# openai/gym

Measured on AMD Instinct MI355X. Metric: env-steps/sec at num_envs=2^20, CartPole-v1, higher is better.
Workload: dtype f64

## Files before the change

### gym_amd/_native.py

```python
from __future__ import annotations

import ctypes as C
import os
import sys
import weakref

import numpy as np

_HERE = os.path.dirname(os.path.abspath(__file__))
LIB_PATH = os.environ.get("MXV_LIB_PATH") or os.path.join(_HERE, "_lib", "libmxv.so")

CARTPOLE, PENDULUM, ACROBOT, MOUNTAINCAR, MOUNTAINCAR_CONT = range(5)
FLAG_ACTION_I32 = 1
FLAG_REWARD_F32 = 2
FLAG_NO_AUTORESET = 4
OK = 0
ERR_INVALID_ARG = -1
ERR_HIP = -2
ERR_INVALID_ACTION = -3
ERR_RESET_NEEDED = -4
ERR_UNSUPPORTED = -5
MAX_PARAMS = 12
ENV_ALIGN = 4
ROLLOUT_EAGER, ROLLOUT_GRAPH, ROLLOUT_FUSED = 0, 1, 2
TAB_FLAG_COMPACT = 1
TAB_FLAG_GENERAL_KERNEL = 2
TAB_KERNEL_NONE, TAB_KERNEL_GENERAL, TAB_KERNEL_TRAJECTORY = 0, 1, 2
COMM_ID_BYTES = 128

EXPORTS = (
    "mxv_env_dims", "mxv_default_params", "mxv_default_reset_bounds", "mxv_version", "mxv_create", "mxv_destroy",
    "mxv_last_error", "mxv_seed", "mxv_seed_actions", "mxv_reset", "mxv_step", "mxv_step_sampled", "mxv_rollout",
    "mxv_rollout_tape", "mxv_sample_actions", "mxv_last_launch", "mxv_last_launch_snapshot", "mxv_reset_host", "mxv_step_host", "mxv_get_state", "mxv_set_state", "mxv_get_counters",
    "mxv_set_counters", "mxv_set_device_clock", "mxv_set_obs_partials", "mxv_set_return_partials", "mxv_obs_partials_layout", "mxv_get_episodes", "mxv_set_episodes", "mxv_get_params", "mxv_set_params", "mxv_set_params_per_env", "mxv_get_params_per_env", "mxv_episode_stats", "mxv_set_episode_outputs", "mxv_episode_stats_host", "mxv_set_running_returns", "mxv_sync", "mxv_get_stream", "mxv_set_stream",
    "mxv_rollout_mixed", "mxv_set_final_snapshot", "mxv_comm_unique_id", "mxv_comm_init", "mxv_comm_destroy", "mxv_allgather_outputs", "mxv_allgather_wait", "mxv_comm_stream",
    "mxv_host_io", "mxv_step_mapped", "mxv_reset_mapped", "mxv_final_packed", "mxv_final_packed_view", "mxv_final_packed_stats_view", "mxv_write_probe", "mxv_write_probe_env", "mxv_host_alloc", "mxv_host_free",
                "mxv_host_block_layout", "mxv_step_host_block", "mxv_wait_stream", "mxv_staging_view", "mxv_adopt_obs",
    "mxv_norm_create", "mxv_norm_destroy", "mxv_norm_last_error", "mxv_norm_set_stream", "mxv_norm_get_state",
    "mxv_norm_set_state", "mxv_norm_observations", "mxv_norm_rewards", "mxv_norm_obs_sums", "mxv_norm_obs_sums_partials", "mxv_norm_reward_sums_partials", "mxv_norm_returns_ptr", "mxv_norm_obs_apply",
    "mxv_norm_reward_sums", "mxv_norm_reward_apply",
    "mxv_subnorm_create", "mxv_subnorm_destroy", "mxv_subnorm_last_error", "mxv_subnorm_set_stream", "mxv_subnorm_get_state",
    "mxv_subnorm_set_state", "mxv_subnorm_observations", "mxv_subnorm_rewards",
    "mxv_tab_create", "mxv_tab_destroy", "mxv_tab_last_error", "mxv_tab_seed", "mxv_tab_seed_actions", "mxv_tab_reset",
    "mxv_tab_step", "mxv_tab_rollout", "mxv_tab_rollout_tape", "mxv_tab_reset_host", "mxv_tab_step_host", "mxv_tab_get_state",
    "mxv_tab_set_state", "mxv_tab_episode_stats", "mxv_tab_set_episode_outputs", "mxv_tab_episode_stats_host",
    "mxv_bj_episode_stats", "mxv_bj_set_episode_outputs", "mxv_bj_episode_stats_host", "mxv_tab_set_running_returns", "mxv_bj_set_running_returns", "mxv_tab_get_counters", "mxv_tab_set_counters", "mxv_tab_sync", "mxv_tab_last_kernel", "mxv_tab_word_threshold", "mxv_tab_set_device_clock", "mxv_bj_set_device_clock", "mxv_tab_set_stream",
    "mxv_get_beyond", "mxv_set_beyond",
    "mxv_bj_create", "mxv_bj_destroy", "mxv_bj_last_error", "mxv_bj_seed", "mxv_bj_reset", "mxv_bj_step", "mxv_bj_rollout", "mxv_bj_rollout_compact",
    "mxv_bj_reset_host", "mxv_bj_step_host", "mxv_bj_get_state", "mxv_bj_set_state", "mxv_bj_get_counters", "mxv_bj_sync", "mxv_bj_set_stream",
    "mxv_placed_alloc", "mxv_placed_free", "mxv_placed_info_get", "mxv_placed_last_error", "mxv_hbm_pair_probe",
)


class MxvLaunchInfo(C.Structure):
    _fields_ = [(k, C.c_int32) for k in ("kernel", "env_id", "param_mode", "envs_per_lane", "safe", "out_mode", "tape", "steps")] + \
               [("grid", C.c_uint32), ("block", C.c_uint32)]
# ... 100 lines not shown
        raise ImportError(
            f"{LIB_PATH} is missing: build the HIP extension first (python -c 'import __graft_entry__ as g; g.build()' "
            "or gym_amd/csrc/build.sh). gym_amd has no CPU fallback."
        )
    _share_torch_hip_runtime()
    lib = C.CDLL(LIB_PATH)
    vp, i32, i64, u64, u32 = C.c_void_p, C.c_int32, C.c_int64, C.c_uint64, C.c_uint32
    sig = {
        "mxv_env_dims": ([i32, C.POINTER(i32), C.POINTER(i32), C.POINTER(i32)], C.c_int),
        "mxv_default_params": ([i32, vp], C.c_int),
        "mxv_default_reset_bounds": ([i32, vp], C.c_int),
        "mxv_version": ([], C.c_char_p),
        "mxv_create": ([C.POINTER(MxvConfig), C.POINTER(vp)], C.c_int),
        "mxv_seed": ([vp, u64, vp], C.c_int),
        "mxv_seed_actions": ([vp, u64], C.c_int),
        "mxv_reset": ([vp, vp, vp, vp], C.c_int),
        "mxv_step": ([vp, vp, vp, vp, vp, vp, vp], C.c_int),
        "mxv_step_sampled": ([vp, vp, vp, vp, vp, vp, vp], C.c_int),
        "mxv_rollout": ([vp, i32, i32, i32, vp, vp, vp, vp, vp, vp], C.c_int),
        "mxv_rollout_tape": ([vp, i32, i32, vp, vp, vp, vp, vp, vp], C.c_int),
        "mxv_sample_actions": ([vp, vp], C.c_int),
        "mxv_last_launch": ([vp, C.POINTER(MxvLaunchInfo)], C.c_int),
        "mxv_last_launch_snapshot": ([vp, C.POINTER(i32), C.POINTER(i32)], C.c_int),
        "mxv_reset_host": ([vp, vp, vp, vp], C.c_int),
        "mxv_step_host": ([vp, vp, vp, vp, vp, vp, vp], C.c_int),
        "mxv_get_state": ([vp, vp, vp], C.c_int),
        "mxv_adopt_obs": ([vp, vp], C.c_int),
        "mxv_set_state": ([vp, vp, vp], C.c_int),
        "mxv_set_counters": ([vp, u64, u32], C.c_int),
        "mxv_set_obs_partials": ([vp, vp], C.c_int),
        "mxv_set_return_partials": ([vp, vp, C.c_double, vp], C.c_int),
        "mxv_obs_partials_layout": ([vp, C.POINTER(i64), C.POINTER(i64), C.POINTER(i32)], C.c_int),
        "mxv_rollout_mixed": ([vp, C.c_int32, C.c_int32, C.c_int32, vp], C.c_int),
        "mxv_set_final_snapshot": ([vp, vp, vp, vp, vp], C.c_int),
        "mxv_write_probe": ([C.c_int32, i64, C.c_int32, C.c_int32, vp, vp, vp, vp, vp, C.POINTER(C.c_double)], C.c_int),
        "mxv_write_probe_env": ([C.c_int32, C.c_int32, C.c_int32, i64, C.c_int32, C.c_int32, vp, vp, vp, vp, vp, C.POINTER(C.c_double)], C.c_int),
        "mxv_wait_stream": ([vp, vp], C.c_int),
        "mxv_staging_view": ([vp] + [C.POINTER(vp)] * 4, C.c_int),
        "mxv_host_alloc": ([C.c_size_t, C.POINTER(vp)], C.c_int),
        "mxv_host_free": ([vp], C.c_int),
        "mxv_host_block_layout": ([vp] + [C.POINTER(C.c_size_t)] * 6, C.c_int),
        "mxv_step_host_block": ([vp, vp, vp, C.c_int32], C.c_int),
        "mxv_final_packed": ([vp, C.c_int32, C.POINTER(C.c_int32)], C.c_int),
        "mxv_final_packed_stats_view": ([vp, C.POINTER(vp), C.POINTER(vp)], C.c_int),
        "mxv_final_packed_view": ([vp, C.POINTER(vp), C.POINTER(vp), C.POINTER(vp)], C.c_int),
        "mxv_comm_unique_id": ([vp], C.c_int),
# ... 485 lines not shown

    def get_state(self):
        st = np.empty((self.S, self.num_envs), dtype=np.float64)
        el = np.empty(self.num_envs, dtype=np.int32)
        self._check(lib.mxv_get_state(self._h, st.ctypes.data, el.ctypes.data))
        return st, el

    def set_state(self, state=None, elapsed=None):
        st = None if state is None else np.ascontiguousarray(state, dtype=np.float64)
        el = None if elapsed is None else np.ascontiguousarray(elapsed, dtype=np.int32)
        if st is not None:
            assert st.shape == (self.S, self.num_envs), st.shape
        if el is not None:
            assert el.shape == (self.num_envs,)
        self._check(lib.mxv_set_state(self._h, _ptr(st), _ptr(el)))

    def last_launch(self) -> dict:
        info = MxvLaunchInfo()
        self._check(lib.mxv_last_launch(self._h, C.byref(info)))
        out = {k: int(getattr(info, k)) for k, _ in MxvLaunchInfo._fields_}
        out["snapshot"] = int(self._final_snapshot()[1])
        return out

    def _final_snapshot(self):
        attached, deposited = C.c_int32(), C.c_int32()
        self._check(lib.mxv_last_launch_snapshot(self._h, C.byref(attached), C.byref(deposited)))
        return bool(attached.value), bool(deposited.value)

    @property
    def final_snapshot_attached(self) -> bool:
        return self._final_snapshot()[0]

    def set_counters(self, t: int, r: int):
        self._check(lib.mxv_set_counters(self._h, int(t), int(r)))

    def set_obs_partials(self, partials_dev=None):
        self._check(lib.mxv_set_obs_partials(self._h, _ptr(partials_dev)))

    def set_return_partials(self, returns_state_ptr=None, gamma: float = 0.99, partials_dev=None):
        self._check(lib.mxv_set_return_partials(self._h, _ptr(returns_state_ptr), float(gamma), _ptr(partials_dev)))

    def obs_partials_layout(self):
        lv, per, vals = C.c_int64(), C.c_int64(), C.c_int32()
        self._check(lib.mxv_obs_partials_layout(self._h, C.byref(lv), C.byref(per), C.byref(vals)))
        return lv.value, per.value, vals.value

# ... 527 lines not shown
```

### gym_amd/csrc/mxv_api.cpp

```cpp
#include <hip/hip_runtime.h>
#include <dlfcn.h>
#include <rccl/rccl.h>

#include <algorithm>
#include <cmath>
#include <cstdlib>
#include <cstring>
#include <map>
#include <new>
#include <string>
#include <tuple>
#include <vector>

#include "mxv_host.hpp"
#include "mxv_kernels.hpp"
#include "mxv_render.hpp"
#include "../../include/mxv_render.h"

using namespace mxv;

namespace {

constexpr int kStateDim[MXV_NUM_ENV_KINDS] = {4, 2, 4, 2, 2};
constexpr int kObsDim[MXV_NUM_ENV_KINDS] = {4, 3, 6, 2, 2};
// ... 34 lines not shown

}

struct mxv_handle : mxv::HostCore {
    static constexpr const char *kNullMessage = "NULL handle";
    mxv_handle() : HostCore("mxv") {}
    mxv_config cfg{};
    int S = 0, O = 0, NA = 0;
    double *state = nullptr;
    float *adopted_obs = nullptr;
    int32_t *lo = nullptr;
    bool hilo = false;
    void *elapsed = nullptr;
    bool elapsed16 = false;
    uint32_t *episodes = nullptr;
    double *ret_state = nullptr, *ret_part = nullptr;
    double ret_gamma = 0.0;
    double *obs_part = nullptr;
    uint32_t *clock_ticket = nullptr;
    bool state_injected = false;
    bool state_out_of_range = false;
    LaunchInfo last_launch{-1, 0, 0, 0, 0, 0, 0, 0, 0, 0};
    bool last_launch_snapshot = false;
    bool step_noise = false;
    EnvParams P{};
    bool default_params = true;
    uint8_t *beyond = nullptr;
    double *params_pe = nullptr;
    int param_mode() const { return params_pe ? PM_PER_ENV : (default_params ? PM_DEFAULT : PM_BROADCAST); }
    double bounds[2] = {0, 0};
    void *st_actions = nullptr;
    float *st_obs = nullptr, *st_final = nullptr;
    void *st_reward = nullptr;
    uint8_t *st_term = nullptr, *st_trunc = nullptr, *st_mask = nullptr;
    void *hm_block = nullptr;
    void *dv_block = nullptr;
    size_t io_total = 0, io_out_off = 0, io_out_bytes = 0, io_act_bytes = 0;
    int32_t *hm_err = nullptr;
    bool hostmap = false;
    char *fin_dev = nullptr;
    char *fin_host = nullptr;
    bool err_in_block = false;
    size_t fin_last = 0;
    bool fin_packed = false;
    using GraphKey = std::tuple<int, int, void *, void *, void *, void *, void *, void *>;
    std::map<GraphKey, hipGraphExec_t> graphs;
// ... 54 lines not shown
    a.state = h->state;
    a.elapsed = h->elapsed;
    a.elapsed16 = h->elapsed16 ? 1 : 0;
    a.episodes = h->episodes;
    a.seeds = h->seeds;
    a.t_dev = nullptr;
    a.err = h->err_in_block ? h->hm_err : h->err;
    a.n = h->cfg.num_envs;
    a.env0 = (uint64_t)h->cfg.env_offset;
    a.base_seed = h->base_seed;
    a.action_seed = h->action_seed;
    a.t = h->t;
    if (h->dev_clock) {
        a.t_dev = h->t_dev;
        a.t = 0;
    }
    a.b0 = h->bounds[0];
    a.b1 = h->bounds[1];
    a.max_steps = h->cfg.max_episode_steps;
    a.flags = h->cfg.flags;
    a.K = 1;
    a.state_injected = (h->state_injected || h->state_out_of_range) ? 1 : 0;
    a.step_noise = h->step_noise ? 1 : 0;
    a.slice = 0;
    a.act_slice = 0;
    a.params_pe = h->params_pe;
    a.beyond = h->beyond;
    a.ep_acc = h->ep_acc;
    a.ep_return_out = h->ep_acc ? h->ep_return_out : nullptr;
    a.ep_length_out = h->ep_acc ? h->ep_length_out : nullptr;
    a.snap_obs = nullptr;
    a.snap_reward = nullptr;
    a.snap_terminated = a.snap_truncated = nullptr;
    a.P = h->P;
}

int track_source(mxv_handle *h, const void *actions, int64_t row, int32_t K, const float **src) {
    *src = nullptr;
    if (!h->last_u) return MXV_OK;
    if (actions) {
        *src = (const float *)actions + row * h->cfg.num_envs;
        return MXV_OK;
    }
    SampleArgs a{};
    a.actions_out = h->blit_actions;
    a.t_dev = h->dev_clock ? h->t_dev : nullptr;
// ... 83 lines not shown
    fill_step_args(h, a);
    a.actions = actions;
    a.actions_out = actions_out;
    a.obs = obs;
    a.reward = reward;
    a.terminated = term;
    a.truncated = trunc;
    a.final_obs = final_obs;
    const bool self_clock = h->dev_clock && h->cfg.num_envs <= kClockInKernelEnvs && h->param_mode() == PM_DEFAULT && !hilo_step;
    if (self_clock) {
        a.clock_out = h->t_dev;
        a.clock_ticket = h->clock_ticket;
    }
    if (int rc = check_step_buffers(h, a)) return rc;
    const float *track = nullptr;
    if (int rc = track_source(h, actions, 0, 1, &track)) return rc;
    if (hilo_step) {
        a.hi_in = h->adopted_obs;
        a.lo = h->lo;
        MXV_HIP(h, launch_hilo_step(h->cfg.env_id, a, h->stream, &h->last_launch));
    } else {
        MXV_HIP(h, launch_step(h->cfg.env_id, h->param_mode(), a, h->stream, &h->last_launch));
    }
    h->last_launch_snapshot = false;
    h->state_injected = false;
    if (int rc = track_step(h, track)) return rc;
    if (self_clock) {
        h->t += 1;
        return MXV_OK;
    }
    return clock_add(h, 1);
}

int parse_bounds(mxv_handle *h, const double *b, double *out) {
    if (!b) {
        default_bounds(h->cfg.env_id, out);
        return MXV_OK;
    }
    if (std::isnan(b[0]) || std::isnan(b[1])) return fail(h, MXV_ERR_INVALID_ARG, "reset bounds are NaN");
    if (h->cfg.env_id != MXV_PENDULUM && b[0] > b[1])
        return fail(h, MXV_ERR_INVALID_ARG, "Lower bound (%g) must be lower than higher bound (%g).", b[0], b[1]);
    out[0] = b[0];
    out[1] = b[1];
    return MXV_OK;
}

// ... 338 lines not shown
    if (h->obs_part || h->ret_part) {
        a.obs_part = h->obs_part;
        if (h->ret_part) {
            a.ret_part = h->ret_part;
            a.ret_state = h->ret_state;
            a.ret_gamma = h->ret_gamma;
        }
        if (!launch_step_supports_stats(h->cfg.env_id, h->param_mode(), a))
            return fail(h, MXV_ERR_UNSUPPORTED, "partial sums are attached (mxv_set_obs_partials / mxv_set_return_partials), but this launch cannot produce them: they "
                                                "exist for sampled [K][N] trajectory launches (K >= 2) with every per-step output, default physics "
                                                "parameters, autoreset and a state the engine produced itself; detach (NULL) and use mxv_norm_obs_sums / mxv_norm_reward_sums");
    }
    const bool in_kernel = h->snap_obs && launch_step_is_rollout(h->param_mode(), a);
    if (in_kernel) {
        a.snap_obs = h->snap_obs;
        a.snap_reward = h->snap_reward;
        a.snap_terminated = h->snap_term;
        a.snap_truncated = h->snap_trunc;
    }
    if (int rc = check_step_buffers(h, a)) return rc;
    const float *track = nullptr;
    if (int rc = track_source(h, actions_tape, K - 1, K, &track)) return rc;
    MXV_HIP(h, launch_step(h->cfg.env_id, h->param_mode(), a, h->stream, &h->last_launch));
    h->last_launch_snapshot = a.snap_obs != nullptr;
    h->state_injected = false;
    if (int rc = track_step(h, track)) return rc;
    if (int rc = clock_add(h, K)) return rc;
    if (h->snap_obs && !in_kernel) return copy_final_snapshot(h, K, per_step, obs, reward, term, trunc);
    return MXV_OK;
}

}

extern "C" {

int mxv_rollout(mxv_handle *h, int32_t K, int32_t per_step, int32_t mode, void *actions_out_dev, float *obs_dev,
                void *reward_dev, uint8_t *terminated_dev, uint8_t *truncated_dev, float *final_obs_dev) {
    MXV_CHECK(h);
    if (int rc = rollout_checks(h, K, obs_dev)) return rc;
    if (mode == MXV_ROLLOUT_FUSED)
        return fused_launch(h, K, per_step, nullptr, actions_out_dev, obs_dev, reward_dev, terminated_dev,
                            truncated_dev, final_obs_dev);
    if (mode != MXV_ROLLOUT_EAGER && mode != MXV_ROLLOUT_GRAPH) return fail(h, MXV_ERR_INVALID_ARG, "unknown rollout mode %d", mode);
    if (int rc = no_partials_here(h, "a rollout of single-step launches (MXV_ROLLOUT_EAGER / _GRAPH)")) return rc;
    const size_t n = (size_t)h->cfg.num_envs;
    auto slice = [&](void *p, size_t elem_bytes, int k) -> void * {
        if (!p) return nullptr;
        return per_step ? (void *)((char *)p + (size_t)k * n * elem_bytes) : p;
    };
    {
        StepArgs a0{};
        fill_step_args(h, a0);
        a0.actions_out = actions_out_dev; a0.obs = obs_dev; a0.reward = reward_dev; a0.final_obs = final_obs_dev;
        if (int rc = check_step_buffers(h, a0)) return rc;
    }
    auto launch_k = [&](int k, const uint64_t *t_dev, uint64_t t) -> hipError_t {
        StepArgs a{};
        fill_step_args(h, a);
        a.t_dev = t_dev;
        a.t = t;
        a.actions = nullptr;
        a.actions_out = slice(actions_out_dev, h->action_bytes(), k);
        a.obs = (float *)slice(obs_dev, h->O * sizeof(float), k);
        a.reward = slice(reward_dev, h->reward_bytes(), k);
        a.terminated = (uint8_t *)slice(terminated_dev, 1, k);
        a.truncated = (uint8_t *)slice(truncated_dev, 1, k);
        a.final_obs = (float *)slice(final_obs_dev, h->O * sizeof(float), k);
        a.ep_return_out = (float *)slice(a.ep_return_out, sizeof(float), k);
        a.ep_length_out = (int32_t *)slice(a.ep_length_out, sizeof(int32_t), k);
        return launch_step(h->cfg.env_id, h->param_mode(), a, h->stream, &h->last_launch);
    };
    const float *track = nullptr;
    if (int rc = track_source(h, nullptr, 0, K, &track)) return rc;
    hipStreamCaptureStatus capturing = hipStreamCaptureStatusNone;
    (void)hipStreamIsCapturing(h->stream, &capturing);
    if (mode == MXV_ROLLOUT_EAGER || capturing != hipStreamCaptureStatusNone) {
        for (int k = 0; k < K; ++k)
            MXV_HIP(h, launch_k(k, h->dev_clock ? h->t_dev : nullptr, h->dev_clock ? (uint64_t)k : h->t + (uint64_t)k));
    } else {
        mxv_handle::GraphKey key{K, per_step, actions_out_dev, obs_dev, reward_dev, terminated_dev, truncated_dev,
                                 final_obs_dev};
        auto it = h->graphs.find(key);
        if (it == h->graphs.end()) {
            hipGraph_t graph = nullptr;
            MXV_HIP(h, hipStreamBeginCapture(h->stream, hipStreamCaptureModeThreadLocal));
            hipError_t le = hipSuccess;
            for (int k = 0; k < K && le == hipSuccess; ++k) le = launch_k(k, h->t_dev, (uint64_t)k);
            hipError_t ce = hipStreamEndCapture(h->stream, &graph);
            if (le != hipSuccess || ce != hipSuccess) {
                if (graph) (void)hipGraphDestroy(graph);
                return fail(h, MXV_ERR_HIP, "graph capture: %s", hipGetErrorString(le != hipSuccess ? le : ce));
            }
// ... 354 lines not shown
                    in_range = false;
                    break;
                }
        }
        h->state_injected = !in_range;
        h->state_out_of_range = !in_range && h->cfg.env_id == MXV_PENDULUM;
    }
    return MXV_OK;
}

int mxv_last_launch(mxv_handle *h, mxv_launch_info *out) {
    MXV_CHECK(h);
    if (!out) return fail(h, MXV_ERR_INVALID_ARG, "mxv_last_launch: out is NULL");
    static_assert(sizeof(mxv_launch_info) == sizeof(LaunchInfo), "mxv_launch_info mirrors LaunchInfo member for member");
    std::memcpy(out, &h->last_launch, sizeof(*out));
    return MXV_OK;
}

int mxv_last_launch_snapshot(mxv_handle *h, int32_t *attached, int32_t *deposited) {
    MXV_CHECK(h);
    if (!attached && !deposited) return fail(h, MXV_ERR_INVALID_ARG, "mxv_last_launch_snapshot: both outputs are NULL");
    if (attached) *attached = h->snap_obs != nullptr ? 1 : 0;
    if (deposited) *deposited = h->last_launch_snapshot ? 1 : 0;
    return MXV_OK;
}

int mxv_get_counters(mxv_handle *h, uint64_t *t, uint32_t *r) {
    MXV_CHECK(h);
    return get_counters(h, t, r);
}

int mxv_set_counters(mxv_handle *h, uint64_t t, uint32_t r) {
    MXV_CHECK(h);
    return set_counters(h, t, r);
}

int mxv_set_obs_partials(mxv_handle *h, double *partials_dev) {
    MXV_CHECK(h);
    h->obs_part = partials_dev;
    return MXV_OK;
}

int mxv_set_return_partials(mxv_handle *h, double *returns_state_dev, double gamma, double *partials_dev) {
    MXV_CHECK(h);
    if (partials_dev && !returns_state_dev) return fail(h, MXV_ERR_INVALID_ARG, "mxv_set_return_partials: the running returns [N] are required");
    h->ret_part = partials_dev;
// ... 597 lines not shown
```

### gym_amd/csrc/mxv_kernels.hip

```cpp
#include <cstdlib>
#include <type_traits>

#include "mxv_host.hpp"
#include "mxv_kernels.hpp"

namespace mxv {

namespace {

__device__ __forceinline__ void raise_error(int32_t *err, int32_t bit) { *reinterpret_cast<volatile int32_t *>(err) = bit; }

typedef float f32x4_t __attribute__((ext_vector_type(4)));
typedef float f32x2_t __attribute__((ext_vector_type(2)));
typedef int i32x4_t __attribute__((ext_vector_type(4)));
typedef int i32x2_t __attribute__((ext_vector_type(2)));
template <bool NT, typename T>
__device__ __forceinline__ void st(T *p, T v) {
    if constexpr (NT) __builtin_nontemporal_store(v, p);
    else *p = v;
}
__device__ __forceinline__ int32_t load_elapsed(const void *p, int32_t el16, int64_t e) {
    return el16 ? (int32_t) static_cast<const uint16_t *>(p)[e] : static_cast<const int32_t *>(p)[e];
}
template <bool NT = false>
__device__ __forceinline__ void store_elapsed(void *p, int32_t el16, int64_t e, int32_t v) {
    if (el16)
        st<NT>(static_cast<uint16_t *>(p) + e, (uint16_t)(v > 65535 ? 65535 : v));
    else
        st<NT>(static_cast<int32_t *>(p) + e, v);
}

template <int O, bool NT = false>
__device__ __forceinline__ void store_obs(float *base, int64_t e, const float *o) {
    if constexpr (O == 4) {
        st<NT>(reinterpret_cast<f32x4_t *>(base) + e, f32x4_t{o[0], o[1], o[2], o[3]});
    } else if constexpr (O == 2) {
        st<NT>(reinterpret_cast<f32x2_t *>(base) + e, f32x2_t{o[0], o[1]});
    } else if constexpr (O == 6) {
        float2 *p = reinterpret_cast<float2 *>(base) + e * 3;
        p[0] = make_float2(o[0], o[1]);
        p[1] = make_float2(o[2], o[3]);
        p[2] = make_float2(o[4], o[5]);
    } else {
        float *p = base + e * O;
#pragma unroll
        for (int k = 0; k < O; ++k) p[k] = o[k];
    }
}

__device__ __forceinline__ uint32_t pin32(uint32_t v) {
    asm volatile("" : "+v"(v));
    return v;
}

template <int O>
// ... 47 lines not shown
template <int O>
__device__ __forceinline__ void load_obs(const float *base, int64_t e, float *o) {
    if constexpr (O == 4) {
        const f32x4_t v = reinterpret_cast<const f32x4_t *>(base)[e];
        o[0] = v.x; o[1] = v.y; o[2] = v.z; o[3] = v.w;
    } else if constexpr (O == 2) {
        const f32x2_t v = reinterpret_cast<const f32x2_t *>(base)[e];
        o[0] = v.x; o[1] = v.y;
    } else {
#pragma unroll
        for (int k = 0; k < O; ++k) o[k] = base[e * O + k];
    }
}
template <int S>
__device__ __forceinline__ void load_lo(const int32_t *base, int64_t e, int32_t *v) {
    if constexpr (S == 4) {
        const i32x4_t q = reinterpret_cast<const i32x4_t *>(base)[e];
        v[0] = q.x; v[1] = q.y; v[2] = q.z; v[3] = q.w;
    } else {
        const i32x2_t q = reinterpret_cast<const i32x2_t *>(base)[e];
        v[0] = q.x; v[1] = q.y;
    }
}
template <int S, bool NT = false>
__device__ __forceinline__ void store_lo(int32_t *base, int64_t e, const int32_t *v) {
    if constexpr (S == 4)
        st<NT>(reinterpret_cast<i32x4_t *>(base) + e, i32x4_t{v[0], v[1], v[2], v[3]});
    else
        st<NT>(reinterpret_cast<i32x2_t *>(base) + e, i32x2_t{v[0], v[1]});
}
template <int ENV>
__global__ void __launch_bounds__(kBlock) hilo_split_kernel(const double *state, float *hi_obs, int32_t *lo, double *side, int64_t n) {
    constexpr int S = Env<ENV>::S;
    static_assert(Env<ENV>::O == S, "the observation must be float32(state), component by component");
    const int64_t e = (int64_t)blockIdx.x * kBlock + threadIdx.x;
    if (e >= n) return;
    static_assert(S == 2 || S == 4, "row accesses of the int32 halves");
    float o[S];
    int32_t l[S];
#pragma unroll
    for (int k = 0; k < S; ++k) {
        const double x = state[(int64_t)k * n + e];
        o[k] = (float)x;
        l[k] = hilo_encode(x, side + (int64_t)k * n + e);
    }
    store_obs<S>(hi_obs, e, o);
    store_lo<S>(lo, e, l);
}
template <int ENV>
__global__ void __launch_bounds__(kBlock) hilo_join_kernel(const float *hi_obs, const int32_t *lo, double *state, int64_t n) {
    constexpr int S = Env<ENV>::S;
    const int64_t e = (int64_t)blockIdx.x * kBlock + threadIdx.x;
    if (e >= n) return;
    float o[S];
    int32_t l[S];
    load_obs<S>(hi_obs, e, o);
    load_lo<S>(lo, e, l);
#pragma unroll
    for (int k = 0; k < S; ++k) state[(int64_t)k * n + e] = hilo_decode(o[k], l[k], state + (int64_t)k * n + e);
}

template <int ENV, int DEF, int E, bool MULTI, bool CLOCK = false, bool HILO = false>
__global__ void __launch_bounds__(kBlock, 1) step_kernel(const StepArgs a) {
    using EV = Env<ENV>;
    constexpr int S = EV::S, O = EV::O, NA = EV::NA;
    static_assert(!HILO || (!MULTI && S == O && EV::AUX == 0), "HILO: one step, observation = float32(state)");
    constexpr int TILE = E * kBlock;
    constexpr bool NT = !MULTI;
    const int tid = threadIdx.x;
    const int64_t tile0 = (int64_t)xcd_contiguous_tile(blockIdx.x, gridDim.x) * TILE;
    const int64_t n = a.n;
    const Par<DEF> P(a.P, a.params_pe, a.n);
    const uint64_t t0 = a.t + (a.t_dev ? *a.t_dev : 0);
    const bool autoreset = !(a.flags & MXV_FLAG_NO_AUTORESET);
    const bool sampled = a.actions == nullptr;
    auto env_of = [&](int j) -> int64_t { return tile0 + (int64_t)j * kBlock + tid; };

    constexpr int AUXN = EV::AUX > 0 ? EV::AUX : 1;
    double s[E][S], aux[E][AUXN];
    int32_t el[E];
    bool valid[E];
#pragma unroll
    for (int j = 0; j < E; ++j) {
        const int64_t e = env_of(j);
        valid[j] = e < n;
        const int64_t ec = valid[j] ? e : 0;
        if constexpr (HILO) {
            float hi[O];
            int32_t l[S];
            load_obs<O>(a.hi_in, ec, hi);
            load_lo<S>(a.lo, ec, l);
// ... 140 lines not shown
                const U4 w = episode_reset_words(seed, k_reset);
                double ns[S], naux[AUXN];
                float nobs[O];
                EV::reset(w, a.b0, a.b1, ns);
                EV::observe(ns, nobs, naux);
#pragma unroll
                for (int j = 0; j < E; ++j)
                    if (j == jsel) {
#pragma unroll
                        for (int k = 0; k < EV::AUX; ++k) aux[j][k] = naux[k];
#pragma unroll
                        for (int k = 0; k < S; ++k) s[j][k] = ns[k];
#pragma unroll
                        for (int k = 0; k < O; ++k) obs[j][k] = nobs[k];
                        el[j] = 0;
                        if constexpr (!LAZY_EP) ep[j] += 1;
                        pend[j] = false;
                    }
            }
        }

#pragma unroll
        for (int j = 0; j < E; ++j) {
            if (!valid[j]) continue;
            const int64_t e = so + env_of(j);
            store_obs<O, NT>(a.obs, e, obs[j]);
            if (a.reward != nullptr) {
                if (a.flags & MXV_FLAG_REWARD_F32)
                    st<NT>(static_cast<float *>(a.reward) + e, (float)rew[j]);
                else
                    st<NT>(static_cast<double *>(a.reward) + e, rew[j]);
            }
            if (a.terminated != nullptr) st<NT>(a.terminated + e, (uint8_t)(term[j] ? 1 : 0));
            if (a.truncated != nullptr) st<NT>(a.truncated + e, (uint8_t)(trunc[j] ? 1 : 0));
        }
        if constexpr (ENV == MXV_CARTPOLE) {
            if (a.beyond != nullptr) {
#pragma unroll
                for (int j = 0; j < E; ++j)
                    if (valid[j] && term[j]) {
                        uint8_t *mark = a.beyond + env_of(j);
                        if (landed((uint32_t)*mark) == 0u) {
                            *mark = 1;
                        } else if (a.reward != nullptr) {
                            if (a.flags & MXV_FLAG_REWARD_F32)
                                static_cast<float *>(a.reward)[so + env_of(j)] = 0.0f;
                            else
                                static_cast<double *>(a.reward)[so + env_of(j)] = 0.0;
                        }
                    }
            }
        }
    }

#pragma unroll
    for (int j = 0; j < E; ++j) {
        if (!valid[j]) continue;
        const int64_t e = env_of(j);
        if constexpr (HILO) {
            int32_t l[S];
            bool esc = false;
#pragma unroll
            for (int k = 0; k < S; ++k) {
                l[k] = hilo_encode_fast(s[j][k]);
                esc = esc || l[k] == kHiloEscape;
            }
            if (__builtin_expect(__any(esc), 0)) {
#pragma unroll
                for (int k = 0; k < S; ++k)
                    if (l[k] == kHiloEscape) a.state[(int64_t)k * n + e] = s[j][k];
            }
            store_lo<S, NT>(a.lo, e, l);
        } else {
#pragma unroll
            for (int k = 0; k < S; ++k) st<NT>(a.state + (int64_t)k * n + e, s[j][k]);
        }
        store_elapsed<NT>(a.elapsed, a.elapsed16, e, el[j]);
        if (ep[j] != ep_in[j]) a.episodes[e] = ep[j];
        if (a.ep_acc) a.ep_acc[e] = er[j];
    }
    if constexpr (CLOCK) {
        if (tid == 0) {
            const uint32_t ticket = atomicAdd(a.clock_ticket, 1u);
            if (ticket == gridDim.x - 1) {
                *a.clock_ticket = 0u;
                *a.clock_out = t0 - a.t + (uint64_t)a.K;
            }
        }
    }
}

constexpr int kWave = 64;
constexpr int kSimds = 1024;

template <int S, int O, int AUX>
// ... 638 lines not shown
        if (out == 2) return launch_rollout_out<ENV, DEF, ER, SAFE, 2>(grid, stream, a, info);
    }
    launch_rollout_out<ENV, DEF, ER, SAFE, 0>(grid, stream, a, info);
}

constexpr int stats_envs_per_lane(int env_id) { return env_id == MXV_ACROBOT ? 1 : 2; }
template <int ENV>
hipError_t launch_rollout_stats(const StepArgs &a, hipStream_t stream, LaunchInfo *info) {
    constexpr int SE = stats_envs_per_lane(ENV);
    const int64_t rtile = (int64_t)SE * kWave;
    const unsigned grid = (unsigned)((a.n + rtile - 1) / rtile);
    const int st = (a.obs_part != nullptr ? 1 : 0) | (a.ret_part != nullptr ? 2 : 0);
    const bool compact = (a.flags & (MXV_FLAG_REWARD_F32 | MXV_FLAG_ACTION_I32)) != 0;
    if (st == 1 && !compact) launch_rollout_out<ENV, true, SE, false, 1, false, 1>(grid, stream, a, info);
    else if (st == 1) launch_rollout_out<ENV, true, SE, false, 2, false, 1>(grid, stream, a, info);
    else if (st == 2 && !compact) launch_rollout_out<ENV, true, SE, false, 1, false, 2>(grid, stream, a, info);
    else if (st == 2) launch_rollout_out<ENV, true, SE, false, 2, false, 2>(grid, stream, a, info);
    else if (!compact) launch_rollout_out<ENV, true, SE, false, 1, false, 3>(grid, stream, a, info);
    else launch_rollout_out<ENV, true, SE, false, 2, false, 3>(grid, stream, a, info);
    return hipGetLastError();
}

constexpr int64_t kStepOneEnvPerLaneFrom = (int64_t)1 << 19;

template <int ENV>
hipError_t launch_step_env(int pm, const StepArgs &a, hipStream_t stream, LaunchInfo *info) {
    const bool def = pm == PM_DEFAULT;
    if ((a.obs_part != nullptr || a.ret_part != nullptr) && launch_step_supports_stats(ENV, pm, a)) return launch_rollout_stats<ENV>(a, stream, info);
    if (launch_step_is_rollout(pm, a)) {
        const bool bounded = ENV != MXV_PENDULUM || (a.max_steps > 0 && a.max_steps < 1000000);
        const bool fast = def && !a.state_injected && bounded;
        auto go = [&](auto er_tag) {
            constexpr int ER = decltype(er_tag)::value;
            const int64_t rtile = (int64_t)ER * kWave;
            const unsigned rgrid = (unsigned)((a.n + rtile - 1) / rtile);
            if (!def) {
                launch_rollout<ENV, false, ER, true>(rgrid, stream, a, info);
            } else if (fast) {
                launch_rollout<ENV, true, ER, false>(rgrid, stream, a, info);
            } else {
                launch_rollout<ENV, true, ER, true>(rgrid, stream, a, info);
            }
        };
        constexpr int ER = rollout_envs_per_lane(ENV);
        if (ER > 1 && a.n <= (int64_t)kSimds * ER * kWave)
            go(std::integral_constant<int, 1>{});
        else
            go(std::integral_constant<int, ER>{});
        return hipGetLastError();
    }
    constexpr int E = envs_per_lane(ENV);
    const int64_t tile = (int64_t)E * kBlock;
    const unsigned grid = (unsigned)((a.n + tile - 1) / tile);
    if (info) *info = LaunchInfo{0, ENV, pm, E, 1, 0, a.actions != nullptr ? 1 : 0, a.K, grid, (uint32_t)kBlock};
    if constexpr (ENV == MXV_CARTPOLE && E > 1) {
        if (a.K == 1 && pm == PM_DEFAULT && a.clock_ticket == nullptr && a.n >= kStepOneEnvPerLaneFrom) {
            const unsigned grid1 = (unsigned)((a.n + kBlock - 1) / kBlock);
            if (info) *info = LaunchInfo{0, ENV, pm, 1, 1, 0, a.actions != nullptr ? 1 : 0, a.K, grid1, (uint32_t)kBlock};
            hipLaunchKernelGGL((step_kernel<ENV, PM_DEFAULT, 1, false>), dim3(grid1), dim3(kBlock), 0, stream, a);
            return hipGetLastError();
        }
    }
    if (a.K > 1) {
        if (pm == PM_DEFAULT)
            hipLaunchKernelGGL((step_kernel<ENV, PM_DEFAULT, E, true>), dim3(grid), dim3(kBlock), 0, stream, a);
        else if (pm == PM_BROADCAST)
            hipLaunchKernelGGL((step_kernel<ENV, PM_BROADCAST, E, true>), dim3(grid), dim3(kBlock), 0, stream, a);
        else
            hipLaunchKernelGGL((step_kernel<ENV, PM_PER_ENV, E, true>), dim3(grid), dim3(kBlock), 0, stream, a);
    } else {
        if (pm == PM_DEFAULT && a.clock_ticket != nullptr)
            hipLaunchKernelGGL((step_kernel<ENV, PM_DEFAULT, E, false, true>), dim3(grid), dim3(kBlock), 0, stream, a);
        else if (pm == PM_DEFAULT)
            hipLaunchKernelGGL((step_kernel<ENV, PM_DEFAULT, E, false>), dim3(grid), dim3(kBlock), 0, stream, a);
        else if (pm == PM_BROADCAST)
            hipLaunchKernelGGL((step_kernel<ENV, PM_BROADCAST, E, false>), dim3(grid), dim3(kBlock), 0, stream, a);
        else
            hipLaunchKernelGGL((step_kernel<ENV, PM_PER_ENV, E, false>), dim3(grid), dim3(kBlock), 0, stream, a);
    }
    return hipGetLastError();
}

// ... 1 lines not shown
hipError_t launch_sample_env(int pm, const SampleArgs &a, hipStream_t stream) {
    const int64_t groups = (a.n + 3) / 4;
    const unsigned grid = (unsigned)((groups + kBlock - 1) / kBlock);
    if (pm == PM_DEFAULT)
        hipLaunchKernelGGL((sample_kernel<ENV, PM_DEFAULT>), dim3(grid), dim3(kBlock), 0, stream, a);
    else if (pm == PM_BROADCAST)
        hipLaunchKernelGGL((sample_kernel<ENV, PM_BROADCAST>), dim3(grid), dim3(kBlock), 0, stream, a);
    else
        hipLaunchKernelGGL((sample_kernel<ENV, PM_PER_ENV>), dim3(grid), dim3(kBlock), 0, stream, a);
    return hipGetLastError();
}

}

bool hilo_supported(int env_id) { return env_id == MXV_CARTPOLE || env_id == MXV_MOUNTAINCAR || env_id == MXV_MOUNTAINCAR_CONT; }

template <int ENV>
static hipError_t launch_hilo_step_env(const StepArgs &a, hipStream_t stream, LaunchInfo *info) {
    constexpr int E = envs_per_lane(ENV);
    if constexpr (ENV == MXV_CARTPOLE && E > 1) {
        if (a.n >= kStepOneEnvPerLaneFrom) {
            const unsigned grid1 = (unsigned)((a.n + kBlock - 1) / kBlock);
            if (info) *info = LaunchInfo{0, ENV, PM_DEFAULT, 1, 1, 3, a.actions != nullptr ? 1 : 0, 1, grid1, (uint32_t)kBlock};
            hipLaunchKernelGGL((step_kernel<ENV, PM_DEFAULT, 1, false, false, true>), dim3(grid1), dim3(kBlock), 0, stream, a);
            return hipGetLastError();
        }
    }
    const int64_t tile = (int64_t)E * kBlock;
    const unsigned grid = (unsigned)((a.n + tile - 1) / tile);
    if (info) *info = LaunchInfo{0, ENV, PM_DEFAULT, E, 1, 3 , a.actions != nullptr ? 1 : 0, 1, grid, (uint32_t)kBlock};
    hipLaunchKernelGGL((step_kernel<ENV, PM_DEFAULT, E, false, false, true>), dim3(grid), dim3(kBlock), 0, stream, a);
    return hipGetLastError();
}
hipError_t launch_hilo_step(int env_id, const StepArgs &a, hipStream_t stream, LaunchInfo *info) {
    switch (env_id) {
        case MXV_CARTPOLE: return launch_hilo_step_env<MXV_CARTPOLE>(a, stream, info);
        case MXV_MOUNTAINCAR: return launch_hilo_step_env<MXV_MOUNTAINCAR>(a, stream, info);
        case MXV_MOUNTAINCAR_CONT: return launch_hilo_step_env<MXV_MOUNTAINCAR_CONT>(a, stream, info);
        default: return hipErrorInvalidValue;
    }
}
hipError_t launch_hilo_split(int env_id, const double *state, float *hi_obs, int32_t *lo, double *side, int64_t n, hipStream_t stream) {
    const dim3 grid((unsigned)((n + kBlock - 1) / kBlock)), block(kBlock);
    switch (env_id) {
        case MXV_CARTPOLE: hipLaunchKernelGGL(hilo_split_kernel<MXV_CARTPOLE>, grid, block, 0, stream, state, hi_obs, lo, side, n); break;
        case MXV_MOUNTAINCAR: hipLaunchKernelGGL(hilo_split_kernel<MXV_MOUNTAINCAR>, grid, block, 0, stream, state, hi_obs, lo, side, n); break;
        case MXV_MOUNTAINCAR_CONT: hipLaunchKernelGGL(hilo_split_kernel<MXV_MOUNTAINCAR_CONT>, grid, block, 0, stream, state, hi_obs, lo, side, n); break;
        default: return hipErrorInvalidValue;
    }
    return hipGetLastError();
}
hipError_t launch_hilo_join(int env_id, const float *hi_obs, const int32_t *lo, double *state, int64_t n, hipStream_t stream) {
    const dim3 grid((unsigned)((n + kBlock - 1) / kBlock)), block(kBlock);
    switch (env_id) {
        case MXV_CARTPOLE: hipLaunchKernelGGL(hilo_join_kernel<MXV_CARTPOLE>, grid, block, 0, stream, hi_obs, lo, state, n); break;
        case MXV_MOUNTAINCAR: hipLaunchKernelGGL(hilo_join_kernel<MXV_MOUNTAINCAR>, grid, block, 0, stream, hi_obs, lo, state, n); break;
        case MXV_MOUNTAINCAR_CONT: hipLaunchKernelGGL(hilo_join_kernel<MXV_MOUNTAINCAR_CONT>, grid, block, 0, stream, hi_obs, lo, state, n); break;
        default: return hipErrorInvalidValue;
    }
    return hipGetLastError();
}

bool launch_step_is_rollout(int pm, const StepArgs &a) {
    const bool sampled_or_tape = a.actions == nullptr || (a.act_slice != 0 && pm == PM_DEFAULT);
    return sampled_or_tape && !(a.flags & MXV_FLAG_NO_AUTORESET) && a.K > 1 && pm != PM_PER_ENV && !a.step_noise;
}

bool launch_step_supports_stats(int env_id, int pm, const StepArgs &a) {
    if (!launch_step_is_rollout(pm, a) || pm != PM_DEFAULT || a.actions != nullptr || a.state_injected) return false;
    if (env_id == MXV_PENDULUM && !(a.max_steps > 0 && a.max_steps < 1000000)) return false;
    if (!(a.reward && a.actions_out && a.terminated && a.truncated && !a.final_obs && !a.ep_acc) || a.slice == 0) return false;
    const int f = a.flags & (MXV_FLAG_REWARD_F32 | MXV_FLAG_ACTION_I32);
    return f == 0 || f == (MXV_FLAG_REWARD_F32 | MXV_FLAG_ACTION_I32);
}
int64_t stats_leaf_envs(int env_id) {
    switch (env_id) {
        case MXV_CARTPOLE: return (int64_t)stats_envs_per_lane(MXV_CARTPOLE) * kWave;
        case MXV_PENDULUM: return (int64_t)stats_envs_per_lane(MXV_PENDULUM) * kWave;
        case MXV_ACROBOT: return (int64_t)stats_envs_per_lane(MXV_ACROBOT) * kWave;
        case MXV_MOUNTAINCAR: return (int64_t)stats_envs_per_lane(MXV_MOUNTAINCAR) * kWave;
        default: return (int64_t)stats_envs_per_lane(MXV_MOUNTAINCAR_CONT) * kWave;
    }
}

hipError_t launch_step(int env_id, int default_params, const StepArgs &a, hipStream_t stream, LaunchInfo *info) {
// ... 148 lines not shown
```

### gym_amd/csrc/mxv_kernels.hpp

```cpp
#pragma once
#include <hip/hip_runtime.h>
#include <stdint.h>

#include "mxv_device.hpp"

namespace mxv {

struct StepArgs {
    double *state;
    void *elapsed;
    uint32_t *episodes;
    const void *actions;
    void *actions_out;
    float *obs;
    void *reward;
    uint8_t *terminated;
    uint8_t *truncated;
    float *final_obs;
    const uint64_t *seeds;
    const uint64_t *t_dev;
    double *ret_state;
    double *ret_part;
    double ret_gamma;
    double *obs_part;
    uint64_t *clock_out;
    uint32_t *clock_ticket;
    int32_t *err;
    int64_t n;
    uint64_t env0;
    uint64_t base_seed;
    uint64_t action_seed;
    uint64_t t;
    double b0, b1;
    int32_t max_steps;
    int32_t flags;
    int32_t K;
    int32_t state_injected;
    int32_t elapsed16;
    const float *hi_in;
    int32_t *lo;
    int32_t step_noise;
    int64_t slice;
    int64_t act_slice;
    const double *params_pe;
    uint8_t *beyond;
    float *ep_acc;
    float *ep_return_out;
    int32_t *ep_length_out;
    float *snap_obs;
    void *snap_reward;
    uint8_t *snap_terminated;
    uint8_t *snap_truncated;
    EnvParams P;
};

struct MixedArgs {
    StepArgs seg[MXV_MAX_MIXED];
    uint32_t first_block[MXV_MAX_MIXED + 1];
    int32_t kind[MXV_MAX_MIXED];
    int32_t count;
};

struct ResetArgs {
    double *state;
// ... 41 lines not shown
constexpr int envs_per_lane(int env_id) { return kStepEnvsPerLane[env_id]; }
constexpr int kRolloutEnvsPerLane[MXV_NUM_ENV_KINDS] = {2, 1, 1, 2, 2};
constexpr int rollout_envs_per_lane(int env_id) { return kRolloutEnvsPerLane[env_id]; }
constexpr int kRolloutPassPeriod = 8;
constexpr int kBlock = 256;

struct LaunchInfo {
    int32_t kernel;
    int32_t env_id;
    int32_t param_mode;
    int32_t envs_per_lane;
    int32_t safe;
    int32_t out_mode;
    int32_t tape;
    int32_t steps;
    uint32_t grid, block;
};
hipError_t launch_step(int env_id, int param_mode, const StepArgs &a, hipStream_t stream, LaunchInfo *info = nullptr);
bool hilo_supported(int env_id);
hipError_t launch_hilo_step(int env_id, const StepArgs &a, hipStream_t stream, LaunchInfo *info = nullptr);
hipError_t launch_hilo_split(int env_id, const double *state, float *hi_obs, int32_t *lo, double *side, int64_t n, hipStream_t stream);
hipError_t launch_hilo_join(int env_id, const float *hi_obs, const int32_t *lo, double *state, int64_t n, hipStream_t stream);
bool launch_step_is_rollout(int param_mode, const StepArgs &a);
bool launch_step_supports_stats(int env_id, int param_mode, const StepArgs &a);
int64_t stats_leaf_envs(int env_id);
hipError_t launch_reset(int env_id, const ResetArgs &a, hipStream_t stream);
hipError_t launch_sample(int env_id, int param_mode, const SampleArgs &a, hipStream_t stream);
hipError_t launch_mixed_rollout(const MixedArgs &m, hipStream_t stream);
int64_t compact_chunks(int64_t n);
hipError_t launch_compact_final(int obs_dim, const CompactArgs &a, hipStream_t stream);
hipError_t launch_write_probe(float *obs, double *rew, int64_t *act, uint8_t *term, uint8_t *trunc, int64_t n, int K, hipStream_t stream);
hipError_t launch_write_probe_env(int env_id, int flags, float *obs, void *rew, void *act, uint8_t *term, uint8_t *trunc, int64_t n, int K,
                                  hipStream_t stream);

}
```

### include/mxv_diag.h

```cpp
#ifndef MXV_DIAG_H
#define MXV_DIAG_H

#include "mxv.h"

#ifdef __cplusplus
extern "C" {
#endif

typedef struct mxv_launch_info {
    int32_t kernel;
    int32_t env_id;
    int32_t param_mode;
    int32_t envs_per_lane;
    int32_t safe;
    int32_t out_mode;
    int32_t tape;
    int32_t steps;
    uint32_t grid, block;
} mxv_launch_info;
int mxv_last_launch(mxv_handle *h, mxv_launch_info *out);
int mxv_last_launch_snapshot(mxv_handle *h, int32_t *attached, int32_t *deposited);


int mxv_write_probe(int32_t device, int64_t num_envs, int32_t K, int32_t launches, float *obs_dev, double *reward_dev, int64_t *actions_dev,
                    uint8_t *terminated_dev, uint8_t *truncated_dev, double *us_per_step);

int mxv_write_probe_env(int32_t device, int32_t env_id, int32_t flags, int64_t num_envs, int32_t K, int32_t launches, float *obs_dev,
                        void *reward_dev, void *actions_dev, uint8_t *terminated_dev, uint8_t *truncated_dev, double *us_per_step);

typedef struct mxv_placed mxv_placed;
#define MXV_PLACED_CHUNK_BYTES ((size_t)256 << 20)
#define MXV_PLACED_MIN_BYTES ((size_t)2 << 30)
enum { MXV_PLACED_PLAIN = 1, MXV_PLACED_NO_JUMP = 2 };
typedef struct mxv_placed_info {
    int32_t placed;
    int32_t balanced;
    int32_t chunks_created;
    int32_t chunks_kept;
    int32_t classes_seen;
    int32_t class_chunks[4];
    int32_t solo_group;
    int32_t solo_class;
    int32_t stop_reason;
    double same_class_us;
// ... 16 lines not shown
```

Baseline: 186.5 billion.

## Use paired 16-byte write-through stores for CartPole single-step outputs

```diff
diff --git a/gym_amd/_native.py b/gym_amd/_native.py
--- a/gym_amd/_native.py
+++ b/gym_amd/_native.py
@@ -31,7 +31,7 @@
 EXPORTS = (
     "mxv_env_dims", "mxv_default_params", "mxv_default_reset_bounds", "mxv_version", "mxv_create", "mxv_destroy",
     "mxv_last_error", "mxv_seed", "mxv_seed_actions", "mxv_reset", "mxv_step", "mxv_step_sampled", "mxv_rollout",
-    "mxv_rollout_tape", "mxv_sample_actions", "mxv_last_launch", "mxv_last_launch_snapshot", "mxv_reset_host", "mxv_step_host", "mxv_get_state", "mxv_set_state", "mxv_get_counters",
+    "mxv_rollout_tape", "mxv_sample_actions", "mxv_last_launch", "mxv_last_launch_snapshot", "mxv_last_launch_store_form", "mxv_reset_host", "mxv_step_host", "mxv_get_state", "mxv_set_state", "mxv_get_counters",
     "mxv_set_counters", "mxv_set_device_clock", "mxv_set_obs_partials", "mxv_set_return_partials", "mxv_obs_partials_layout", "mxv_get_episodes", "mxv_set_episodes", "mxv_get_params", "mxv_set_params", "mxv_set_params_per_env", "mxv_get_params_per_env", "mxv_episode_stats", "mxv_set_episode_outputs", "mxv_episode_stats_host", "mxv_set_running_returns", "mxv_sync", "mxv_get_stream", "mxv_set_stream",
     "mxv_rollout_mixed", "mxv_set_final_snapshot", "mxv_comm_unique_id", "mxv_comm_init", "mxv_comm_destroy", "mxv_allgather_outputs", "mxv_allgather_wait", "mxv_comm_stream",
     "mxv_host_io", "mxv_step_mapped", "mxv_reset_mapped", "mxv_final_packed", "mxv_final_packed_view", "mxv_final_packed_stats_view", "mxv_write_probe", "mxv_write_probe_env", "mxv_host_alloc", "mxv_host_free",
@@ -178,6 +178,7 @@
         "mxv_sample_actions": ([vp, vp], C.c_int),
         "mxv_last_launch": ([vp, C.POINTER(MxvLaunchInfo)], C.c_int),
         "mxv_last_launch_snapshot": ([vp, C.POINTER(i32), C.POINTER(i32)], C.c_int),
+        "mxv_last_launch_store_form": ([vp, C.POINTER(i32), C.POINTER(C.c_int64), C.POINTER(C.c_int64)], C.c_int),
         "mxv_reset_host": ([vp, vp, vp, vp], C.c_int),
         "mxv_step_host": ([vp, vp, vp, vp, vp, vp, vp], C.c_int),
         "mxv_get_state": ([vp, vp, vp], C.c_int),
@@ -709,6 +710,11 @@
         out["snapshot"] = int(self._final_snapshot()[1])
         return out
 
+    def last_launch_store_form(self):
+        wt, frm, upto = C.c_int32(0), C.c_int64(0), C.c_int64(0)
+        self._check(lib.mxv_last_launch_store_form(self._h, C.byref(wt), C.byref(frm), C.byref(upto)))
+        return bool(wt.value), int(frm.value), int(upto.value)
+
     def _final_snapshot(self):
         attached, deposited = C.c_int32(), C.c_int32()
         self._check(lib.mxv_last_launch_snapshot(self._h, C.byref(attached), C.byref(deposited)))
diff --git a/gym_amd/csrc/mxv_api.cpp b/gym_amd/csrc/mxv_api.cpp
--- a/gym_amd/csrc/mxv_api.cpp
+++ b/gym_amd/csrc/mxv_api.cpp
@@ -80,6 +80,7 @@
     bool state_out_of_range = false;
     LaunchInfo last_launch{-1, 0, 0, 0, 0, 0, 0, 0, 0, 0};
     bool last_launch_snapshot = false;
+    bool last_launch_write_through = false;
     bool step_noise = false;
     EnvParams P{};
     bool default_params = true;
@@ -180,6 +181,7 @@
     a.K = 1;
     a.state_injected = (h->state_injected || h->state_out_of_range) ? 1 : 0;
     a.step_noise = h->step_noise ? 1 : 0;
+    a.host_io = h->hostmap ? 1 : 0;
     a.slice = 0;
     a.act_slice = 0;
     a.params_pe = h->params_pe;
@@ -309,6 +311,7 @@
     } else {
         MXV_HIP(h, launch_step(h->cfg.env_id, h->param_mode(), a, h->stream, &h->last_launch));
     }
+    h->last_launch_write_through = launch_step_writes_through(h->cfg.env_id, h->param_mode(), a);
     h->last_launch_snapshot = false;
     h->state_injected = false;
     if (int rc = track_step(h, track)) return rc;
@@ -693,6 +696,7 @@
     const float *track = nullptr;
     if (int rc = track_source(h, actions_tape, K - 1, K, &track)) return rc;
     MXV_HIP(h, launch_step(h->cfg.env_id, h->param_mode(), a, h->stream, &h->last_launch));
+    h->last_launch_write_through = launch_step_writes_through(h->cfg.env_id, h->param_mode(), a);
     h->last_launch_snapshot = a.snap_obs != nullptr;
     h->state_injected = false;
     if (int rc = track_step(h, track)) return rc;
@@ -739,6 +743,7 @@
         a.final_obs = (float *)slice(final_obs_dev, h->O * sizeof(float), k);
         a.ep_return_out = (float *)slice(a.ep_return_out, sizeof(float), k);
         a.ep_length_out = (int32_t *)slice(a.ep_length_out, sizeof(int32_t), k);
+        h->last_launch_write_through = launch_step_writes_through(h->cfg.env_id, h->param_mode(), a);
         return launch_step(h->cfg.env_id, h->param_mode(), a, h->stream, &h->last_launch);
     };
     const float *track = nullptr;
@@ -1139,6 +1144,15 @@
     if (!attached && !deposited) return fail(h, MXV_ERR_INVALID_ARG, "mxv_last_launch_snapshot: both outputs are NULL");
     if (attached) *attached = h->snap_obs != nullptr ? 1 : 0;
     if (deposited) *deposited = h->last_launch_snapshot ? 1 : 0;
+    return MXV_OK;
+}
+
+int mxv_last_launch_store_form(mxv_handle *h, int32_t *write_through, int64_t *write_through_from, int64_t *write_through_up_to) {
+    MXV_CHECK(h);
+    if (!write_through && !write_through_from && !write_through_up_to) return fail(h, MXV_ERR_INVALID_ARG, "mxv_last_launch_store_form: every output is NULL");
+    if (write_through) *write_through = h->last_launch_write_through ? 1 : 0;
+    if (write_through_from) *write_through_from = kStepWriteThroughFrom;
+    if (write_through_up_to) *write_through_up_to = kStepWriteThroughUpTo;
     return MXV_OK;
 }
 
diff --git a/gym_amd/csrc/mxv_kernels.hip b/gym_amd/csrc/mxv_kernels.hip
--- a/gym_amd/csrc/mxv_kernels.hip
+++ b/gym_amd/csrc/mxv_kernels.hip
@@ -10,19 +10,47 @@
 
 __device__ __forceinline__ void raise_error(int32_t *err, int32_t bit) { *reinterpret_cast<volatile int32_t *>(err) = bit; }
 
+enum { ST_PLAIN = 0, ST_NT = 1, ST_WT = 2 };
 typedef float f32x4_t __attribute__((ext_vector_type(4)));
 typedef float f32x2_t __attribute__((ext_vector_type(2)));
 typedef int i32x4_t __attribute__((ext_vector_type(4)));
 typedef int i32x2_t __attribute__((ext_vector_type(2)));
-template <bool NT, typename T>
+typedef double f64x2_t __attribute__((ext_vector_type(2)));
+template <typename T>
+__device__ __forceinline__ void st_wt16(T *p, T v) {
+    static_assert(sizeof(T) == 16, "write-through stores are 16 bytes per lane");
+    i32x4_t q;
+    __builtin_memcpy(&q, &v, 16);
+    asm volatile("global_store_dwordx4 %0, %1, off sc1\n\ts_nop 1" ::"v"(p), "v"(q) : "memory");
+}
+template <int SP, typename T>
 __device__ __forceinline__ void st(T *p, T v) {
-    if constexpr (NT) __builtin_nontemporal_store(v, p);
+    if constexpr (SP == ST_WT && sizeof(T) == 16) st_wt16(p, v);
+    else if constexpr (SP != ST_PLAIN) __builtin_nontemporal_store(v, p);
     else *p = v;
+}
+__device__ __forceinline__ double pair_swap(double v) {
+    int2 w;
+    __builtin_memcpy(&w, &v, 8);
+    w.x = __builtin_amdgcn_mov_dpp(w.x, 0xB1, 0xF, 0xF, true);
+    w.y = __builtin_amdgcn_mov_dpp(w.y, 0xB1, 0xF, 0xF, true);
+    double r;
+    __builtin_memcpy(&r, &w, 8);
+    return r;
+}
+__device__ __forceinline__ void st_wt_pair(double *px, double *py, int64_t e, bool odd, double x, double y) {
+    const double got = pair_swap(odd ? x : y);
+    double *p = odd ? py + (e - 1) : px + e;
+    st_wt16(reinterpret_cast<f64x2_t *>(p), odd ? f64x2_t{got, y} : f64x2_t{x, got});
+}
+__device__ __forceinline__ void st_wt_even(double *p, int64_t e, bool odd, double v) {
+    const double got = pair_swap(v);
+    if (!odd) st_wt16(reinterpret_cast<f64x2_t *>(p + e), f64x2_t{v, got});
 }
 __device__ __forceinline__ int32_t load_elapsed(const void *p, int32_t el16, int64_t e) {
     return el16 ? (int32_t) static_cast<const uint16_t *>(p)[e] : static_cast<const int32_t *>(p)[e];
 }
-template <bool NT = false>
+template <int NT = ST_PLAIN>
 __device__ __forceinline__ void store_elapsed(void *p, int32_t el16, int64_t e, int32_t v) {
     if (el16)
         st<NT>(static_cast<uint16_t *>(p) + e, (uint16_t)(v > 65535 ? 65535 : v));
@@ -30,7 +58,7 @@
         st<NT>(static_cast<int32_t *>(p) + e, v);
 }
 
-template <int O, bool NT = false>
+template <int O, int NT = ST_PLAIN>
 __device__ __forceinline__ void store_obs(float *base, int64_t e, const float *o) {
     if constexpr (O == 4) {
         st<NT>(reinterpret_cast<f32x4_t *>(base) + e, f32x4_t{o[0], o[1], o[2], o[3]});
@@ -124,7 +152,7 @@
         v[0] = q.x; v[1] = q.y;
     }
 }
-template <int S, bool NT = false>
+template <int S, int NT = ST_PLAIN>
 __device__ __forceinline__ void store_lo(int32_t *base, int64_t e, const int32_t *v) {
     if constexpr (S == 4)
         st<NT>(reinterpret_cast<i32x4_t *>(base) + e, i32x4_t{v[0], v[1], v[2], v[3]});
@@ -162,13 +190,15 @@
     for (int k = 0; k < S; ++k) state[(int64_t)k * n + e] = hilo_decode(o[k], l[k], state + (int64_t)k * n + e);
 }
 
-template <int ENV, int DEF, int E, bool MULTI, bool CLOCK = false, bool HILO = false>
+template <int ENV, int DEF, int E, bool MULTI, bool CLOCK = false, bool HILO = false, bool WT = false>
 __global__ void __launch_bounds__(kBlock, 1) step_kernel(const StepArgs a) {
     using EV = Env<ENV>;
     constexpr int S = EV::S, O = EV::O, NA = EV::NA;
     static_assert(!HILO || (!MULTI && S == O && EV::AUX == 0), "HILO: one step, observation = float32(state)");
     constexpr int TILE = E * kBlock;
-    constexpr bool NT = !MULTI;
+    static_assert(!WT || (ENV == MXV_CARTPOLE && !MULTI && !CLOCK), "WT: CartPole's plain single step (16-byte rows, the state's components in pairs)");
+    constexpr int NT = MULTI ? ST_PLAIN : (WT ? ST_WT : ST_NT);
+    const bool odd = threadIdx.x & 1;
     const int tid = threadIdx.x;
     const int64_t tile0 = (int64_t)xcd_contiguous_tile(blockIdx.x, gridDim.x) * TILE;
     const int64_t n = a.n;
@@ -355,12 +385,15 @@
 
 #pragma unroll
         for (int j = 0; j < E; ++j) {
+            const bool paired = WT && __all(valid[j]);
             if (!valid[j]) continue;
             const int64_t e = so + env_of(j);
             store_obs<O, NT>(a.obs, e, obs[j]);
             if (a.reward != nullptr) {
                 if (a.flags & MXV_FLAG_REWARD_F32)
                     st<NT>(static_cast<float *>(a.reward) + e, (float)rew[j]);
+                else if (paired)
+                    st_wt_even(static_cast<double *>(a.reward), e, odd, rew[j]);
                 else
                     st<NT>(static_cast<double *>(a.reward) + e, rew[j]);
             }
@@ -388,6 +421,7 @@
 
 #pragma unroll
     for (int j = 0; j < E; ++j) {
+        const bool paired = WT && __all(valid[j]);
         if (!valid[j]) continue;
         const int64_t e = env_of(j);
         if constexpr (HILO) {
@@ -404,6 +438,9 @@
                     if (l[k] == kHiloEscape) a.state[(int64_t)k * n + e] = s[j][k];
             }
             store_lo<S, NT>(a.lo, e, l);
+        } else if (paired) {
+#pragma unroll
+            for (int k = 0; k < S; k += 2) st_wt_pair(a.state + (int64_t)k * n, a.state + (int64_t)(k + 1) * n, e, odd, s[j][k], s[j][k + 1]);
         } else {
 #pragma unroll
             for (int k = 0; k < S; ++k) st<NT>(a.state + (int64_t)k * n + e, s[j][k]);
@@ -1088,6 +1125,13 @@
 }
 
 constexpr int64_t kStepOneEnvPerLaneFrom = (int64_t)1 << 19;
+
+static_assert(kStepWriteThroughFrom >= kStepOneEnvPerLaneFrom, "the write-through form exists for the one-env-per-lane launch");
+bool step_writes_through(int env_id, int pm, const StepArgs &a) {
+    auto aligned16 = [](const void *p) { return (reinterpret_cast<uintptr_t>(p) & 15u) == 0; };
+    return env_id == MXV_CARTPOLE && a.K == 1 && pm == PM_DEFAULT && a.clock_ticket == nullptr && !a.host_io && a.n >= kStepWriteThroughFrom && a.n <= kStepWriteThroughUpTo && a.n % 2 == 0 &&
+           a.beyond == nullptr && aligned16(a.state) && aligned16(a.lo) && aligned16(a.obs) && aligned16(a.reward);
+}
 
 template <int ENV>
 hipError_t launch_step_env(int pm, const StepArgs &a, hipStream_t stream, LaunchInfo *info) {
@@ -1123,7 +1167,10 @@
         if (a.K == 1 && pm == PM_DEFAULT && a.clock_ticket == nullptr && a.n >= kStepOneEnvPerLaneFrom) {
             const unsigned grid1 = (unsigned)((a.n + kBlock - 1) / kBlock);
             if (info) *info = LaunchInfo{0, ENV, pm, 1, 1, 0, a.actions != nullptr ? 1 : 0, a.K, grid1, (uint32_t)kBlock};
-            hipLaunchKernelGGL((step_kernel<ENV, PM_DEFAULT, 1, false>), dim3(grid1), dim3(kBlock), 0, stream, a);
+            if (step_writes_through(ENV, pm, a))
+                hipLaunchKernelGGL((step_kernel<ENV, PM_DEFAULT, 1, false, false, false, true>), dim3(grid1), dim3(kBlock), 0, stream, a);
+            else
+                hipLaunchKernelGGL((step_kernel<ENV, PM_DEFAULT, 1, false>), dim3(grid1), dim3(kBlock), 0, stream, a);
             return hipGetLastError();
         }
     }
@@ -1171,7 +1218,10 @@
         if (a.n >= kStepOneEnvPerLaneFrom) {
             const unsigned grid1 = (unsigned)((a.n + kBlock - 1) / kBlock);
             if (info) *info = LaunchInfo{0, ENV, PM_DEFAULT, 1, 1, 3, a.actions != nullptr ? 1 : 0, 1, grid1, (uint32_t)kBlock};
-            hipLaunchKernelGGL((step_kernel<ENV, PM_DEFAULT, 1, false, false, true>), dim3(grid1), dim3(kBlock), 0, stream, a);
+            if (step_writes_through(ENV, PM_DEFAULT, a))
+                hipLaunchKernelGGL((step_kernel<ENV, PM_DEFAULT, 1, false, false, true, true>), dim3(grid1), dim3(kBlock), 0, stream, a);
+            else
+                hipLaunchKernelGGL((step_kernel<ENV, PM_DEFAULT, 1, false, false, true>), dim3(grid1), dim3(kBlock), 0, stream, a);
             return hipGetLastError();
         }
     }
@@ -1210,6 +1260,7 @@
     return hipGetLastError();
 }
 
+bool launch_step_writes_through(int env_id, int pm, const StepArgs &a) { return step_writes_through(env_id, pm, a); }
 bool launch_step_is_rollout(int pm, const StepArgs &a) {
     const bool sampled_or_tape = a.actions == nullptr || (a.act_slice != 0 && pm == PM_DEFAULT);
     return sampled_or_tape && !(a.flags & MXV_FLAG_NO_AUTORESET) && a.K > 1 && pm != PM_PER_ENV && !a.step_noise;
diff --git a/gym_amd/csrc/mxv_kernels.hpp b/gym_amd/csrc/mxv_kernels.hpp
--- a/gym_amd/csrc/mxv_kernels.hpp
+++ b/gym_amd/csrc/mxv_kernels.hpp
@@ -40,6 +40,7 @@
     const float *hi_in;
     int32_t *lo;
     int32_t step_noise;
+    int32_t host_io;
     int64_t slice;
     int64_t act_slice;
     const double *params_pe;
@@ -127,6 +128,9 @@
 hipError_t launch_hilo_split(int env_id, const double *state, float *hi_obs, int32_t *lo, double *side, int64_t n, hipStream_t stream);
 hipError_t launch_hilo_join(int env_id, const float *hi_obs, const int32_t *lo, double *state, int64_t n, hipStream_t stream);
 bool launch_step_is_rollout(int param_mode, const StepArgs &a);
+constexpr int64_t kStepWriteThroughFrom = (int64_t)7 << 17;
+constexpr int64_t kStepWriteThroughUpTo = (int64_t)3 << 20;
+bool launch_step_writes_through(int env_id, int param_mode, const StepArgs &a);
 bool launch_step_supports_stats(int env_id, int param_mode, const StepArgs &a);
 int64_t stats_leaf_envs(int env_id);
 hipError_t launch_reset(int env_id, const ResetArgs &a, hipStream_t stream);
diff --git a/include/mxv_diag.h b/include/mxv_diag.h
--- a/include/mxv_diag.h
+++ b/include/mxv_diag.h
@@ -20,6 +20,7 @@
 } mxv_launch_info;
 int mxv_last_launch(mxv_handle *h, mxv_launch_info *out);
 int mxv_last_launch_snapshot(mxv_handle *h, int32_t *attached, int32_t *deposited);
+int mxv_last_launch_store_form(mxv_handle *h, int32_t *write_through, int64_t *write_through_from, int64_t *write_through_up_to);
 
 
 int mxv_write_probe(int32_t device, int64_t num_envs, int32_t K, int32_t launches, float *obs_dev, double *reward_dev, int64_t *actions_dev,
```

After: 181.7 billion. 0.975x the previous value.
